# imperatormk/candle-birefnet

Hardware: AMD Instinct MI355X
Metric: images/sec @1024x1024 Swin-L (higher is better)
Workload: dtype f32 storage+accumulate; GEMM operands as two fp16 planes of the power-of-two-scaled operand (22-bit mantissa), 3 fp16 MFMAs/product (fp32-equivalent inside the fp16 range: |GEMM input| < 8190); 1 GPU; BASELINE configs[1]: Swin-L 1024x1024 batch=1 fp32 on 1xMI355X (single-image latency); batch_per_gpu=1, global_batch=1, size=1024, deform_mode=reference_cpu, compute=f32_half2, streams_per_gpu=1, branch_streams_per_gpu=5, inputs=resident in HBM (torch cuda tensors), weights: synthetic seed 42

## Files before the change

### candle_birefnet_amd/_ffi.py

```python
import ctypes as C
import os

_HERE = os.path.dirname(os.path.abspath(__file__))
LIB_PATH = os.environ.get("BRN_LIB_PATH") or os.path.join(_HERE, "libbirefnet_hip.so")

BRN_OK = 0
BRN_MEM_HOST, BRN_MEM_DEVICE = 0, 1
BRN_F32, BRN_F32_SPLIT3, BRN_F32_SPLIT2, BRN_BF16_OPERANDS, BRN_BF16, BRN_BF16_DEC_SPLIT2, BRN_F32_HALF2, BRN_F16 = 0, 1, 2, 3, 4, 5, 6, 7
BRN_DEFORM_REFERENCE_CPU, BRN_DEFORM_DEFORMABLE = 0, 1
BRN_ACT_NONE, BRN_ACT_RELU, BRN_ACT_GELU_ERF = 0, 1, 2

BRN_ERR_INVALID_ARG, BRN_ERR_MISSING_TENSOR, BRN_ERR_SHAPE, BRN_ERR_NO_DEVICE, BRN_ERR_HIP, BRN_ERR_OOM = 1, 2, 3, 4, 5, 6
ERR_NAMES = {1: "INVALID_ARG", 2: "MISSING_TENSOR", 3: "SHAPE", 4: "NO_DEVICE", 5: "HIP", 6: "OOM"}


class BrnError(RuntimeError):

    def __init__(self, status, msg):
        super().__init__(f"[{ERR_NAMES.get(status, status)}] {msg}")
        self.status = status


class brn_config(C.Structure):
    _fields_ = [
# ... 7 lines not shown
        ("deform_mode", C.c_int),
    ]


class brn_named_tensor(C.Structure):
    _fields_ = [("name", C.c_char_p), ("data", C.POINTER(C.c_float)), ("shape", C.POINTER(C.c_int64)), ("ndim", C.c_int)]


def _load():
    if not os.path.exists(LIB_PATH):
        raise ImportError(
            f"{LIB_PATH} not found: build it with `python -c 'import __graft_entry__ as g; g.build()'` "
            "(hipcc --offload-arch=gfx950).  There is no CPU fallback for this package.")
    return C.CDLL(LIB_PATH, mode=C.RTLD_GLOBAL)


lib = _load()

_fp = C.POINTER(C.c_float)
_vp = C.c_void_p


def _sig(name, restype, *argtypes):
    fn = getattr(lib, name)
    fn.restype = restype
    fn.argtypes = list(argtypes)
    return fn


_sig("brn_abi_version", C.c_int)
_sig("brn_last_error", C.c_char_p)
_sig("brn_build_info", C.c_char_p)
_sig("brn_device_count", C.c_int, C.POINTER(C.c_int))
_sig("brn_config_default_swin_l", None, C.POINTER(brn_config))
_sig("brn_config_lateral_channels", None, C.POINTER(brn_config), C.POINTER(C.c_int * 4))
_sig("brn_config_x4_channels", C.c_int, C.POINTER(brn_config))
_sig("brn_model_create", C.c_int, C.POINTER(brn_config), C.POINTER(brn_named_tensor), C.c_size_t, C.c_int, C.c_int,
     C.c_int, C.c_int, C.c_int, C.POINTER(_vp))
_sig("brn_model_create_from_safetensors", C.c_int, C.POINTER(brn_config), C.c_char_p, C.c_char_p, C.c_int, C.c_int, C.c_int,
     C.c_int, C.c_int, C.POINTER(_vp))
_sig("brn_decoder_create", C.c_int, C.POINTER(brn_config), C.POINTER(brn_named_tensor), C.c_size_t, C.c_char_p, C.c_int, C.c_int, C.POINTER(_vp))
_sig("brn_model_destroy", None, _vp)
_sig("brn_forward_logits", C.c_int, _vp, _vp, C.c_int, C.c_int, C.c_int, C.c_int, _vp, C.c_int, _vp)
_sig("brn_forward", C.c_int, _vp, _vp, C.c_int, C.c_int, C.c_int, C.c_int, _vp, C.c_int, _vp)
_sig("brn_model_backbone_forward", C.c_int, _vp, _vp, C.c_int, C.c_int, C.c_int, C.c_int, C.POINTER(_vp), C.c_int, _vp)
_sig("brn_model_squeeze_forward", C.c_int, _vp, _vp, C.c_int, C.c_int, C.c_int, C.c_int, _vp, C.c_int, _vp)
_sig("brn_model_decoder_forward", C.c_int, _vp, _vp, _vp, _vp, _vp, _vp, C.c_int, C.c_int, C.c_int, C.c_int, _vp, C.c_int, _vp)
_sig("brn_model_set_streams", C.c_int, _vp, C.c_int, C.c_int)
_sig("brn_model_set_profiling", C.c_int, _vp, C.c_int)
_sig("brn_model_last_timings", C.c_int, _vp, C.POINTER(C.c_float * 5))
_sig("brn_model_last_kernel_stats", C.c_int, _vp, C.c_int, C.POINTER(C.c_int), C.POINTER(C.c_float), C.POINTER(C.c_double),
     C.POINTER(C.c_double), C.POINTER(C.c_int))
_sig("brn_kernel_family_name", C.c_char_p, C.c_int)
_sig("brn_swin_create", C.c_int, C.POINTER(brn_config), C.POINTER(brn_named_tensor), C.c_size_t, C.c_char_p, C.c_int,
     C.POINTER(_vp))
_sig("brn_swin_destroy", None, _vp)
_sig("brn_swin_forward", C.c_int, _vp, _vp, C.c_int, C.c_int, C.c_int, C.c_int, C.POINTER(_vp), C.c_int, _vp)
_sig("brn_linear_forward", C.c_int, _vp, C.c_int, C.c_int, _vp, _vp, C.c_int, C.c_int, _vp, _vp, C.c_int, C.c_int, _vp)
_sig("brn_linear_residual_layer_norm_forward", C.c_int, _vp, C.c_int, C.c_int, _vp, _vp, C.c_int, _vp, _vp, _vp, C.c_float, _vp, _vp, C.c_int, C.c_int, _vp)
_sig("brn_layer_norm_forward", C.c_int, _vp, C.c_int, C.c_int, _vp, _vp, C.c_float, _vp, C.c_int, C.c_int, _vp)
_sig("brn_conv2d_forward", C.c_int, _vp, C.c_int, C.c_int, C.c_int, C.c_int, _vp, _vp, C.c_int, C.c_int, C.c_int, C.c_int,
     C.c_int, C.c_int, _vp, _vp, _vp, _vp, C.c_float, C.c_int, _vp, C.c_int, C.c_int, _vp)
_sig("brn_upsample_bilinear2d", C.c_int, _vp, C.c_int, C.c_int, C.c_int, C.c_int, C.c_int, C.c_int, _vp, C.c_int, C.c_int, _vp)
_sig("brn_window_attention_forward", C.c_int, _vp, C.c_int, C.c_int, C.c_int, C.c_int, C.c_int, C.c_int, C.c_int, _vp, _vp,
     _vp, _vp, _vp, _vp, C.c_int, C.c_int, _vp)
_sig("brn_patch_merging_forward", C.c_int, _vp, C.c_int, C.c_int, C.c_int, C.c_int, _vp, _vp, _vp, _vp, C.c_int, C.c_int, _vp)
_sig("brn_deform_conv2d_forward", C.c_int, _vp, C.c_int, C.c_int, C.c_int, C.c_int, _vp, _vp, _vp, _vp, _vp, _vp, C.c_int,
     C.c_int, C.c_int, C.c_int, C.c_int, _vp, C.c_int, C.c_int, _vp)

_sig("brn_aspp_deformable_forward", C.c_int, _vp, C.c_size_t, C.c_char_p, C.c_int, C.c_int, C.c_int, _vp, C.c_int, C.c_int, C.c_int, _vp, C.c_int, C.c_int, _vp)

_sig("brn_decblk_forward", C.c_int, _vp, C.c_size_t, C.c_char_p, C.c_int, C.c_int, C.c_int, C.c_int, C.c_int, _vp, C.c_int, C.c_int, C.c_int, _vp, C.c_int,
     C.c_int, _vp)

_sig("brn_preprocess_image", C.c_int, _vp, C.c_int, C.c_int, C.c_int, C.c_int, _vp, C.c_int, C.c_int, _vp)
_sig("brn_postprocess_mask", C.c_int, _vp, C.c_int, C.c_int, C.c_int, C.c_int, C.c_int, _vp, C.c_int, _vp)
_sig("brn_infer_images_u8", C.c_int, _vp, C.c_int, C.POINTER(_vp), C.POINTER(C.c_int), C.POINTER(C.c_int), C.c_int, C.c_int, C.POINTER(_vp), _vp)
_sig("brn_set_op_compute", C.c_int, C.c_int)
if hasattr(lib, "brn_gemm_microbench"):
    _sig("brn_gemm_microbench", C.c_int, C.c_int, C.c_int, C.c_int, C.c_int, C.c_int, C.c_int, C.c_int, C.POINTER(C.c_float))

DECLARED = [
    "brn_abi_version", "brn_last_error", "brn_build_info", "brn_device_count", "brn_config_default_swin_l",
    "brn_config_lateral_channels", "brn_config_x4_channels", "brn_model_create", "brn_model_create_from_safetensors", "brn_decoder_create", "brn_model_destroy", "brn_forward_logits",
    "brn_forward", "brn_model_backbone_forward", "brn_model_squeeze_forward", "brn_model_decoder_forward",
    "brn_model_set_streams", "brn_model_set_profiling", "brn_model_last_timings", "brn_model_last_kernel_stats", "brn_kernel_family_name",
    "brn_swin_create", "brn_swin_destroy", "brn_swin_forward", "brn_linear_forward", "brn_linear_residual_layer_norm_forward", "brn_layer_norm_forward",
    "brn_conv2d_forward", "brn_upsample_bilinear2d", "brn_window_attention_forward", "brn_patch_merging_forward",
    "brn_deform_conv2d_forward", "brn_aspp_deformable_forward", "brn_decblk_forward", "brn_set_op_compute", "brn_preprocess_image", "brn_postprocess_mask", "brn_infer_images_u8",
]


def check(status):
    if status != BRN_OK:
        raise BrnError(status, (lib.brn_last_error() or b"").decode("utf-8", "replace"))


def device_count():
    n = C.c_int(0)
    check(lib.brn_device_count(C.byref(n)))
    return n.value
```

### candle_birefnet_amd/csrc/brn_api.cpp

```cpp
#include "brn_api_util.h"
#include <cstring>
#include <cstdio>
#include <memory>
#include <cstdlib>

namespace brn {

ComputeMode compute_mode(int dt) {
    ComputeMode m;
    if (dt == BRN_F32) m.build.planes = 0;
    else if (dt == BRN_F32_SPLIT3) m.build.planes = 3;
    else if (dt == BRN_F32_SPLIT2) m.build.planes = 2;
    else if (dt == BRN_F32_HALF2) m.build.planes = BUILD_HALF2;
#ifdef BRN_DIAG_BUILD
    else if (dt == BRN_BF16_OPERANDS) m.build.planes = 1;
#else
    else if (dt == BRN_BF16_OPERANDS) fail(BRN_ERR_INVALID_ARG, "compute dtype BRN_BF16_OPERANDS is superseded by BRN_BF16 and only built into libbirefnet_hip_diag.so");
#endif
    else if (dt == BRN_BF16 || dt == BRN_BF16_DEC_SPLIT2 || dt == BRN_F16) { m.build = {BUILD_BF16, dt == BRN_F16}; m.s16 = dt == BRN_F16 ? 2 : 1; }
    else fail(BRN_ERR_INVALID_ARG, "unsupported compute dtype %d", dt);
    return m;
}

static void plan_model(Model& m, int B, int H, int W) {
// ... 340 lines not shown
    delete m;
}

brn_status brn_forward_logits(brn_model* m, const float* x, int B, int H, int W, brn_mem in_loc, float* out, brn_mem out_loc,
                              void* stream) {
    return guarded([&] { run_model(m ? &m->m : nullptr, x, B, H, W, in_loc, out, out_loc, stream, 0); });
}
brn_status brn_forward(brn_model* m, const float* x, int B, int H, int W, brn_mem in_loc, float* out, brn_mem out_loc,
                       void* stream) {
    return guarded([&] { run_model(m ? &m->m : nullptr, x, B, H, W, in_loc, out, out_loc, stream, 1); });
}

brn_status brn_model_set_streams(brn_model* m, int sub_batch_streams, int branch_stream_mask) {
    return guarded([&] {
        if (!m) fail(BRN_ERR_INVALID_ARG, "null model");
        if (sub_batch_streams < 0 || sub_batch_streams > 8 || branch_stream_mask < -1 || branch_stream_mask > 31)
            fail(BRN_ERR_INVALID_ARG, "sub_batch_streams in 0 .. 8 (0 = default), branch_stream_mask in -1 .. 31 (-1 = automatic)");
        std::lock_guard<std::mutex> lk(m->m.mu);
        m->m.opt_parts = sub_batch_streams;
        m->m.opt_branches = branch_stream_mask;
    });
}
brn_status brn_model_set_profiling(brn_model* m, int enable) {
    return guarded([&] {
        if (!m) fail(BRN_ERR_INVALID_ARG, "null model");
        std::lock_guard<std::mutex> lk(m->m.mu);
        m->m.profiling = enable != 0;
    });
}
brn_status brn_model_last_timings(brn_model* m, float ms[5]) {
    return guarded([&] {
        if (!m || !ms) fail(BRN_ERR_INVALID_ARG, "null argument");
        for (int i = 0; i < 5; ++i) ms[i] = m->m.last_ms[i];
    });
}
brn_status brn_model_last_kernel_stats(brn_model* m, int n, int* launches, float* ms, double* flop, double* bytes, int* n_out) {
    return guarded([&] {
        if (!m || !launches || !ms || !flop || !bytes) fail(BRN_ERR_INVALID_ARG, "null argument");
        const int rows = FAM_COUNT + REGION_COUNT;
        const int k = n < rows ? n : rows;
        for (int f = 0; f < k; ++f) {
            launches[f] = m->m.fam_launches[f]; ms[f] = m->m.fam_ms[f]; flop[f] = m->m.fam_flop[f]; bytes[f] = m->m.fam_bytes[f];
        }
        if (n_out) *n_out = rows;
    });
}
const char* brn_kernel_family_name(int f) {
    static const char* names[FAM_COUNT] = {"gemm_dense", "gemm_conv_nhwc", "gemm_gather_nchw", "gemm_deform_nhwc",
                                           "window_attention", "layernorm", "resize", "elementwise"};
    static const char* regions[REGION_COUNT] = {"region_none", "region_aspp"};
    if (f >= FAM_COUNT && f < FAM_COUNT + REGION_COUNT) return regions[f - FAM_COUNT];
    return (f >= 0 && f < FAM_COUNT) ? names[f] : "?";
}

brn_status brn_model_backbone_forward(brn_model* m, const float* x, int B, int H, int W, brn_mem in_loc, float* const outs[4],
                                      brn_mem out_loc, void* stream) {
    return guarded([&] {
        if (!m) fail(BRN_ERR_INVALID_ARG, "null model");
        if (m->m.decoder_only) fail(BRN_ERR_INVALID_ARG, "this handle holds only the decoder (brn_decoder_create)");
        std::lock_guard<std::mutex> lk(m->m.mu);
        swin_entry(m->m.swin, m->m.device, x, B, H, W, in_loc, outs, out_loc, stream, m->m.bf16);
    });
}

brn_status brn_model_squeeze_forward(brn_model* m, const float* x4, int B, int h, int w, brn_mem in_loc, float* out,
                                     brn_mem out_loc, void* stream) {
    return guarded([&] {
        if (!m || !x4 || !out) fail(BRN_ERR_INVALID_ARG, "null argument");
        if (m->m.decoder_only) fail(BRN_ERR_INVALID_ARG, "this handle holds only the decoder (brn_decoder_create)");
        std::lock_guard<std::mutex> lk(m->m.mu);
        BRN_HIP(hipSetDevice(m->m.device));
        const int cin = m->m.squeeze.cin, cout = m->m.squeeze.cout;
        Staging si(stream, in_loc), so(stream, out_loc);
        const float* dx = si.in(x4, (size_t)B * cin * h * w);
        float* dy = so.out(out, (size_t)B * cout * h * w);
        with_arena((hipStream_t)stream, [&](Ctx& c) {
            Map X = new_map(c, B, h, w, cin), Y = new_map(c, B, h, w, cout);
            if (!c.dry) BRN_HIP(launch_nchw_to_nhwc(dx, B, cin, h, w, X.p, X.ld, 0, c.stream, c.bf16));
            decblk_forward(c, m->m.squeeze, X, Y, m->m.cfg.deform_mode);
            if (!c.dry) BRN_HIP(launch_nhwc_to_nchw(Y.p, B, cout, h, w, Y.ld, 0, dy, c.stream, c.bf16));
        }, m->m.dec_bf16);
        so.finish();
    });
}

brn_status brn_model_decoder_forward(brn_model* m, const float* x, const float* x1, const float* x2, const float* x3,
                                     const float* x4, int B, int H, int W, brn_mem in_loc, float* out, brn_mem out_loc,
                                     void* stream) {
    return guarded([&] {
        if (!m || !x || !x1 || !x2 || !x3 || !x4 || !out) fail(BRN_ERR_INVALID_ARG, "null argument");
        if (H % 32 || W % 32 || H < 32 || W < 32) fail(BRN_ERR_INVALID_ARG, "H and W must be positive multiples of 32");
        std::lock_guard<std::mutex> lk(m->m.mu);
        BRN_HIP(hipSetDevice(m->m.device));
        Staging si(stream, in_loc), so(stream, out_loc);
        const int hh[4] = {H / 4, H / 8, H / 16, H / 32}, ww[4] = {W / 4, W / 8, W / 16, W / 32};
        const int ch[4] = {384, 768, 1536, 3072};
        const float* src[4] = {x1, x2, x3, x4};
        const float* dsrc[4];
        for (int i = 0; i < 4; ++i) dsrc[i] = si.in(src[i], (size_t)B * ch[i] * hh[i] * ww[i]);
        const float* dx = si.in(x, (size_t)B * 3 * H * W);
        float* dy = so.out(out, (size_t)B * H * W);
        with_arena((hipStream_t)stream, [&](Ctx& c) {
            Map X1 = new_map(c, B, hh[0], ww[0], 384), X2 = new_map(c, B, hh[1], ww[1], 768), X3 = new_map(c, B, hh[2], ww[2], 1536);
            Map D4 = new_map(c, B, hh[3], ww[3], 3456);
            if (!c.dry) {
                BRN_HIP(launch_nchw_to_nhwc(dsrc[0], B, 384, hh[0], ww[0], X1.p, X1.ld, 0, c.stream, c.bf16));
// ... 12 lines not shown
```

### candle_birefnet_amd/csrc/brn_kernels.h

```cpp
#pragma once
#include <hip/hip_runtime.h>
#include <stdint.h>

namespace brn {

enum GemmMode {
    GEMM_DENSE = 0,
    GEMM_CONV_NHWC = 1,
    GEMM_GATHER_NCHW = 2,
    GEMM_DEFORM_NHWC = 3
};
enum Act { ACT_NONE = 0, ACT_RELU = 1, ACT_GELU_ERF = 2 };

struct GemmParams {
    const float* A;
    const float* W;
    float* C;
    int M, N, K;
    int mode;
    int lda;
    int a_coff;
    int Hin, Win, Cin, kh, kw, stride, pad, dil, Hout, Wout;
    int Kreal;
    const float* om; int om_ld; int om_mask_off;
    int om_sigmoid;
    const float* bias;
    const float* bbias; int bbias_rows;
    const float* scale; const float* shift;
    int act;
    const float* R; int ldr; int r_coff;
    int ldc; int c_coff;
    const void* Wp; int planes; int wp_rows;
    int splitk; float* part;
    int a_planes, c_planes;
    int h2; float a_scale, out_scale;
    int wp_ld;
    int k_chunk_major;
    int c_f32, r_f32;
    int a_bf16, c_bf16;
    unsigned long long* trace;
    int abl;
};

struct GemmPlan { int cfg; int splitk; size_t ws_floats; };
GemmPlan plan_gemm(int M, int N, int K, int planes = 0);
hipError_t launch_gemm(const GemmParams& p, const GemmPlan& plan, float* ws, hipStream_t s);
inline bool gemm_split_is_ws(int cfg) { return cfg == 6 || cfg == 0 || cfg == 3 || cfg == 4 || cfg == 5; }
hipError_t launch_gemm_split(const GemmParams& p, int cfg, hipStream_t s);

int launch_cus();
void set_launch_cus(int n);
GemmPlan plan_gemm_bf16(int M, int N, int K, bool f32_residual = false, bool gelu = false);
hipError_t launch_gemm_bf16(const GemmParams& p, const GemmPlan& plan, float* ws, hipStream_t s);

bool gemm_wstat_eligible(const GemmParams& p);
hipError_t launch_gemm_wstat(const GemmParams& p, hipStream_t s);
bool patch_embed_ln_eligible(int Cin, int N, int k, int stride, int H, int W, int ldw, int ldx);
hipError_t launch_patch_embed_ln(const float* img, int B, int H, int W, const float* wgt, int ldw, const float* bias, const float* gamma,
                                 const float* beta, float eps, float* x, int ldx, hipStream_t s, const float* gamma1 = nullptr,
                                 const float* beta1 = nullptr, void* xn_bf16 = nullptr, int ldxn = 0, int xn_f16 = 0);
bool gemm_wstat_ln_eligible(const GemmParams& p);
bool gemm_rowln_eligible(const GemmParams& p);
hipError_t launch_gemm_rowln(const GemmParams& p, const float* gamma, const float* beta, float eps, void* y_bf16, int ldy, hipStream_t s);
hipError_t launch_gemm_wstat_ln(const GemmParams& p, const float* gamma, const float* beta, float eps, void* y_bf16, int ldy, hipStream_t s);

bool deform_bf16_eligible(const GemmParams& p);
hipError_t launch_deform_bf16(const GemmParams& p, hipStream_t s);

bool gemm_planes_eligible(const GemmParams& p);
GemmPlan plan_gemm_planes(int M, int N, int K, int planes, bool c_planes);
hipError_t launch_gemm_planes(const GemmParams& p, const GemmPlan& plan, float* ws, hipStream_t s);

namespace hf {
GemmPlan plan_gemm_bf16(int M, int N, int K, bool f32_residual = false, bool gelu = false);
hipError_t launch_gemm_bf16(const GemmParams& p, const GemmPlan& plan, float* ws, hipStream_t s);
bool gemm_wstat_eligible(const GemmParams& p);
hipError_t launch_gemm_wstat(const GemmParams& p, hipStream_t s);
bool gemm_wstat_ln_eligible(const GemmParams& p);
hipError_t launch_gemm_wstat_ln(const GemmParams& p, const float* gamma, const float* beta, float eps, void* y_bf16, int ldy, hipStream_t s);
bool gemm_rowln_eligible(const GemmParams& p);
hipError_t launch_gemm_rowln(const GemmParams& p, const float* gamma, const float* beta, float eps, void* y_bf16, int ldy, hipStream_t s);
bool deform_bf16_eligible(const GemmParams& p);
hipError_t launch_deform_bf16(const GemmParams& p, hipStream_t s);
}

#ifdef BRN_DIAG_BUILD
hipError_t launch_mfma_valu_probe(int blocks, int iters, int mode, float* sink, hipStream_t s);
hipError_t launch_lds_mfma_probe(int blocks, int iters, int np, int variant, float* sink, hipStream_t s);
hipError_t launch_mfma_peak_bf16(int blocks, int iters, float* sink, unsigned long long* clk, int nacc, hipStream_t s);
hipError_t launch_mfma_peak(int blocks, int iters, float* sink, unsigned long long* clk, hipStream_t s);
#endif

struct LayerNormParams {
    const float* x; float* y;
    int rows, C;
    const float* gamma; const float* beta; float eps;
    int ldx;
    int ldy, y_coff;
    int mode; int H, W, Cin;
    int y_planes;
    float y_h2;
// ... 53 lines not shown
```

### candle_birefnet_amd/csrc/kernels/gemm_f32.hip

```cpp
#include <cstdlib>
#include "../brn_kernels.h"
#include "gemm_common.h"

namespace brn {

constexpr int LDS_LD = 36;

template <int BM, int BN, int WM, int WN, int MODE>
__global__ void __launch_bounds__(WM* WN * 64) gemm_f32_kernel(const GemmParams p) {
    constexpr int NT = WM * WN * 64;
    constexpr int RPP = NT / 8;
    constexpr int PA = BM / RPP, PB = BN / RPP;
    constexpr int WTM = BM / WM, WTN = BN / WN, TM = WTM / 32, TN = WTN / 32;
    static_assert(PA >= 1 && PB >= 1 && TM >= 1 && TN >= 1, "tile too small for the thread count");

    constexpr int SMEM_MAIN = (BM + BN) * LDS_LD, SMEM_EPI = WM * WN * EPI_WAVE_FLOATS;
    __shared__ __attribute__((aligned(16))) float smem[SMEM_MAIN > SMEM_EPI ? SMEM_MAIN : SMEM_EPI];
    float* As = smem;
    float* Bs = smem + BM * LDS_LD;

    const int tid = threadIdx.x, lane = tid & 63, wave = tid >> 6;
    const int wm = wave / WN, wn = wave % WN;

    const TileSlice ts = tile_slice<BM, BN>(p, BK);
// ... 226 lines not shown
            pl.cfg = 0; pl.splitk = 1; pl.ws_floats = 0;
            static const int sk_t128 = getenv("BRN_SK_T128") ? atoi(getenv("BRN_SK_T128")) : 200;
            if (t128 < sk_t128) {
                int s = (int)(480 / t128);
                if (s > nk / 24) s = nk / 24;
                if (s > 8) s = 8;
                if (s > 1) { pl.splitk = s; pl.ws_floats = (size_t)s * M * N; }
            }
            return pl;
        }
    }
    if (t64 < 384 && nk >= 8) {
        pl.cfg = 2;
        int s = (int)((768 + t64 - 1) / t64);
        if (s > nk / 4) s = nk / 4;
        if (s > 64) s = 64;
        if (s > 1) { pl.splitk = s; pl.ws_floats = (size_t)s * M * N; }
    }
    return pl;
}

static bool deform_on_split(const GemmParams& p) {
    return p.mode == GEMM_DEFORM_NHWC && p.planes >= 2 && p.Wp && p.om && !p.a_bf16 && !p.c_bf16 && (p.Cin % 32) == 0 && p.K == p.kh * p.kw * p.Cin &&
           ((p.lda | p.a_coff) & 3) == 0 && p.Hin + p.pad < 32768 && p.Win + p.pad < 32768 &&
           ((double)p.M / ((double)p.Hout * p.Wout) + 1.0) * p.Hin * p.Win * p.lda * 4.0 < 2147483648.0;
}
static int deform_split_plan(const GemmParams& p, int caller_slices, int& splitk) {
    const GemmPlan pp = plan_gemm(p.M, p.N, p.K, p.planes);
    splitk = pp.splitk < caller_slices ? pp.splitk : caller_slices;
    if (splitk < 1) splitk = 1;
    return gemm_split_is_ws(pp.cfg) ? 0 : 2;
}

hipError_t launch_gemm(const GemmParams& p_in, const GemmPlan& pl, float* ws, hipStream_t s) {
    if (p_in.M <= 0 || p_in.N <= 0 || p_in.K <= 0 || (p_in.K % BK) != 0) return hipErrorInvalidValue;
    if ((p_in.mode == GEMM_CONV_NHWC || p_in.mode == GEMM_DEFORM_NHWC) && (p_in.Cin % BK) != 0) return hipErrorInvalidValue;
    GemmParams p = p_in;
    p.splitk = pl.splitk < 1 ? 1 : pl.splitk;
    p.part = ws;
    if (p.splitk > 1 && !ws) return hipErrorInvalidValue;
    if (p.a_bf16 && p.mode != GEMM_DEFORM_NHWC) return hipErrorInvalidValue;
    if (p.c_bf16 && (p.splitk > 1 || p.R || (p.planes > 0 && p.Wp && p.mode != GEMM_DEFORM_NHWC && p.mode != GEMM_GATHER_NCHW))) return hipErrorInvalidValue;
    const bool deform_split = deform_on_split(p);
    int deform_cfg = 0;
    if (deform_split) deform_cfg = deform_split_plan(p, p.splitk, p.splitk);
    if (p.h2 && !(p.planes == 2 && p.Wp && (p.mode == GEMM_DENSE || p.mode == GEMM_CONV_NHWC || deform_split))) p.h2 = 0;
    if (p.h2 && !(p.a_scale > 0.f && p.out_scale > 0.f)) return hipErrorInvalidValue;
    if (p.a_planes || p.c_planes) {
        if (!(p.planes == 2 || p.planes == 3) || !p.Wp || p.mode != GEMM_DENSE || !gemm_split_is_ws(pl.cfg)) return hipErrorInvalidValue;
        if (p.a_planes && (p.a_planes != p.planes || p.lda % 16 || p.a_coff)) return hipErrorInvalidValue;
        if (p.c_planes && (p.c_planes != p.planes || p.splitk > 1 || p.R || p.N % 32 || p.ldc % 16 || p.c_coff % 32)) return hipErrorInvalidValue;
    }
    hipError_t e;
    if (p.planes > 0 && p.Wp && (p.mode == GEMM_DENSE || p.mode == GEMM_CONV_NHWC)) e = launch_gemm_split(p, pl.cfg, s);
    else if (deform_split) e = launch_gemm_split(p, deform_cfg, s);
    else if (pl.cfg == 0) e = launch_cfg<128, 128, 2, 2>(p, s);
    else if (pl.cfg == 1) e = launch_cfg<128, 64, 2, 2>(p, s);
    else if (pl.cfg == 3) e = launch_cfg<128, 128, 2, 4>(p, s);
    else if (pl.cfg == 4) e = launch_cfg<256, 128, 4, 2>(p, s);
    else if (pl.cfg == 5) e = launch_cfg<128, 128, 4, 2>(p, s);
    else e = launch_cfg<64, 64, 2, 2>(p, s);
    if (e != hipSuccess || p.splitk == 1) return e;
    long total = (long)p.M * p.N;
    long blocks = (total + 255) / 256;
    if (blocks > 4096) blocks = 4096;
    hipLaunchKernelGGL(splitk_reduce_kernel, dim3((unsigned)blocks), dim3(256), 0, s, p);
    return hipGetLastError();
}

}
```

### include/birefnet_hip.h

```cpp
#ifndef BIREFNET_HIP_H
#define BIREFNET_HIP_H

#include <stddef.h>
#include <stdint.h>

#ifdef __cplusplus
extern "C" {
#endif

#define BRN_ABI_VERSION 1

typedef int brn_status;
enum {
    BRN_OK = 0,
    BRN_ERR_INVALID_ARG = 1,
    BRN_ERR_MISSING_TENSOR = 2,
    BRN_ERR_SHAPE = 3,
    BRN_ERR_NO_DEVICE = 4,
    BRN_ERR_HIP = 5,
    BRN_ERR_OOM = 6
};

typedef enum { BRN_MEM_HOST = 0, BRN_MEM_DEVICE = 1 } brn_mem;
typedef enum { BRN_F32 = 0, BRN_F32_SPLIT3 = 1, BRN_F32_SPLIT2 = 2, BRN_BF16_OPERANDS = 3, BRN_BF16 = 4, BRN_BF16_DEC_SPLIT2 = 5, BRN_F32_HALF2 = 6, BRN_F16 = 7 } brn_dtype;
// ... 22 lines not shown
    int deform_mode;
} brn_config;

typedef struct brn_named_tensor {
    const char* name;
    const float* data;
    const int64_t* shape;
    int ndim;
} brn_named_tensor;

typedef struct brn_model brn_model;
typedef struct brn_swin brn_swin;

int brn_abi_version(void);
const char* brn_last_error(void);
brn_status brn_device_count(int* n);
const char* brn_build_info(void);

void brn_config_default_swin_l(brn_config* cfg);
void brn_config_lateral_channels(const brn_config* cfg, int out[4]);
int brn_config_x4_channels(const brn_config* cfg);

brn_status brn_model_create(const brn_config* cfg, const brn_named_tensor* weights, size_t n_weights,
                            int device_ordinal, brn_dtype compute_dtype,
                            int max_batch, int max_h, int max_w, brn_model** out);
brn_status brn_model_create_from_safetensors(const brn_config* cfg, const char* path, const char* prefix,
                                            int device_ordinal, brn_dtype compute_dtype,
                                            int max_batch, int max_h, int max_w, brn_model** out);
void brn_model_destroy(brn_model* m);

brn_status brn_forward_logits(brn_model* m, const float* x_nchw, int B, int H, int W, brn_mem in_loc,
                              float* logits_out, brn_mem out_loc, void* stream);
brn_status brn_forward(brn_model* m, const float* x_nchw, int B, int H, int W, brn_mem in_loc,
                       float* mask_out, brn_mem out_loc, void* stream);

brn_status brn_model_backbone_forward(brn_model* m, const float* x_nchw, int B, int H, int W, brn_mem in_loc,
                                      float* const outs[4], brn_mem out_loc, void* stream);
brn_status brn_model_squeeze_forward(brn_model* m, const float* x4_nchw, int B, int h, int w, brn_mem in_loc,
                                     float* out, brn_mem out_loc, void* stream);
brn_status brn_model_decoder_forward(brn_model* m, const float* x_nchw, const float* x1, const float* x2,
                                     const float* x3, const float* x4, int B, int H, int W, brn_mem in_loc,
                                     float* logits_out, brn_mem out_loc, void* stream);

brn_status brn_decoder_create(const brn_config* cfg, const brn_named_tensor* weights, size_t n_weights, const char* prefix,
                              int device_ordinal, brn_dtype compute_dtype, brn_model** out);

brn_status brn_model_set_streams(brn_model* m, int sub_batch_streams, int branch_stream_mask);

brn_status brn_model_set_profiling(brn_model* m, int enable);
brn_status brn_model_last_timings(brn_model* m, float ms[5]);
brn_status brn_model_last_kernel_stats(brn_model* m, int n, int* launches, float* ms, double* flop,
                                       double* bytes, int* n_out);
const char* brn_kernel_family_name(int f);

brn_status brn_swin_create(const brn_config* cfg , const brn_named_tensor* weights,
                           size_t n_weights, const char* prefix, int device_ordinal, brn_swin** out);
void brn_swin_destroy(brn_swin* s);
brn_status brn_swin_forward(brn_swin* s, const float* x_nchw, int B, int H, int W, brn_mem in_loc,
                            float* const outs[4], brn_mem out_loc, void* stream);

brn_status brn_set_op_compute(int dtype);
brn_status brn_linear_forward(const float* x, int M, int K, const float* w, const float* bias, int N,
                              int act, const float* residual, float* y, brn_mem loc, int device_ordinal,
                              void* stream);
brn_status brn_linear_residual_layer_norm_forward(const float* x, int M, int K, const float* w, const float* bias, int N,
                                                  const float* residual, const float* gamma, const float* beta, float eps,
                                                  float* x_out, float* y_out, brn_mem loc, int device_ordinal, void* stream);

brn_status brn_layer_norm_forward(const float* x, int rows, int C, const float* gamma, const float* beta,
                                  float eps, float* y, brn_mem loc, int device_ordinal, void* stream);
brn_status brn_conv2d_forward(const float* x, int B, int C, int H, int W, const float* w, const float* bias,
                              int O, int kh, int kw, int stride, int pad, int dil,
                              const float* bn_gamma, const float* bn_beta, const float* bn_mean,
                              const float* bn_var, float bn_eps, int act,
                              float* y, brn_mem loc, int device_ordinal, void* stream);
brn_status brn_upsample_bilinear2d(const float* x, int B, int C, int H, int W, int out_h, int out_w,
                                   float* y, brn_mem loc, int device_ordinal, void* stream);
brn_status brn_window_attention_forward(const float* x, int B, int H, int W, int C, int heads, int window_size,
                                        int shift, const float* qkv_w, const float* qkv_b,
                                        const float* proj_w, const float* proj_b, const float* rel_table,
                                        float* y, brn_mem loc, int device_ordinal, void* stream);
brn_status brn_patch_merging_forward(const float* x, int B, int H, int W, int C, const float* norm_g,
                                     const float* norm_b, const float* reduction_w, float* y, brn_mem loc,
                                     int device_ordinal, void* stream);
brn_status brn_deform_conv2d_forward(const float* x, int B, int C, int H, int W,
                                     const float* offset_w, const float* offset_b,
                                     const float* mod_w, const float* mod_b,
                                     const float* w, const float* bias, int O, int k, int stride, int pad,
                                     int mode, float* y, brn_mem loc, int device_ordinal, void* stream);

brn_status brn_aspp_deformable_forward(const brn_named_tensor* weights, size_t n_weights, const char* prefix, int in_channels,
                                       int out_channels, int mode, const float* x, int B, int H, int W, float* y, brn_mem loc,
                                       int device_ordinal, void* stream);

brn_status brn_decblk_forward(const brn_named_tensor* weights, size_t n_weights, const char* prefix, int in_channels,
                              int out_channels, int inter_channels, int use_aspp, int mode, const float* x, int B, int H, int W,
                              float* y, brn_mem loc, int device_ordinal, void* stream);

brn_status brn_preprocess_image(const unsigned char* pixels, int h, int w, int channels, int S,
                                float* x_nchw_out, brn_mem out_loc, int device_ordinal, void* stream);
brn_status brn_postprocess_mask(const float* logits, int S, brn_mem in_loc, int apply_sigmoid, int out_h, int out_w,
                                unsigned char* mask_out, int device_ordinal, void* stream);

brn_status brn_infer_images_u8(brn_model* m, int n, const unsigned char* const* pixels, const int* heights, const int* widths,
                               int channels, int S, unsigned char* const* masks, void* stream);

// ... 5 lines not shown
```

### rust_shim/src/hip_ffi.rs

```rust
#![allow(non_camel_case_types)]
use libc::{c_char, c_double, c_float, c_int, c_uchar, c_void, size_t};

pub const BRN_ABI_VERSION: c_int = 1;
pub const BRN_OK: c_int = 0;
pub const BRN_MEM_HOST: c_int = 0;
pub const BRN_MEM_DEVICE: c_int = 1;
pub const BRN_F32: c_int = 0;
pub const BRN_F32_SPLIT3: c_int = 1;
pub const BRN_F32_SPLIT2: c_int = 2;
pub const BRN_BF16_OPERANDS: c_int = 3;
pub const BRN_BF16: c_int = 4;
pub const BRN_BF16_DEC_SPLIT2: c_int = 5;
pub const BRN_F32_HALF2: c_int = 6;
pub const BRN_F16: c_int = 7;
pub const BRN_DEFORM_REFERENCE_CPU: c_int = 0;
pub const BRN_DEFORM_DEFORMABLE: c_int = 1;
pub const BRN_ACT_NONE: c_int = 0;
pub const BRN_ACT_RELU: c_int = 1;
pub const BRN_ACT_GELU_ERF: c_int = 2;

#[repr(C)]
#[derive(Clone, Copy)]
pub struct BrnConfig {
    pub size_w: c_int,
// ... 11 lines not shown
    pub num_heads: [c_int; 4],
    pub window_size: c_int,
    pub mlp_ratio: c_float,
    pub patch_size: c_int,
    pub in_channels: c_int,
    pub drop_path_rate: c_float,
    pub deform_mode: c_int,
}

#[repr(C)]
pub struct BrnNamedTensor {
    pub name: *const c_char,
    pub data: *const c_float,
    pub shape: *const i64,
    pub ndim: c_int,
}

pub enum BrnModel {}
pub enum BrnSwin {}

extern "C" {
    pub fn brn_abi_version() -> c_int;
    pub fn brn_last_error() -> *const c_char;
    pub fn brn_device_count(n: *mut c_int) -> c_int;
    pub fn brn_build_info() -> *const c_char;
    pub fn brn_config_default_swin_l(cfg: *mut BrnConfig);
    pub fn brn_config_lateral_channels(cfg: *const BrnConfig, out: *mut c_int);
    pub fn brn_config_x4_channels(cfg: *const BrnConfig) -> c_int;
    pub fn brn_model_create(cfg: *const BrnConfig, weights: *const BrnNamedTensor, n_weights: size_t, device_ordinal: c_int,
                            compute_dtype: c_int, max_batch: c_int, max_h: c_int, max_w: c_int, out: *mut *mut BrnModel) -> c_int;
    pub fn brn_model_create_from_safetensors(cfg: *const BrnConfig, path: *const c_char, prefix: *const c_char, device_ordinal: c_int,
                                             compute_dtype: c_int, max_batch: c_int, max_h: c_int, max_w: c_int,
                                             out: *mut *mut BrnModel) -> c_int;
    pub fn brn_decoder_create(cfg: *const BrnConfig, weights: *const BrnNamedTensor, n_weights: size_t, prefix: *const c_char,
                              device_ordinal: c_int, compute_dtype: c_int, out: *mut *mut BrnModel) -> c_int;
    pub fn brn_model_destroy(m: *mut BrnModel);
    pub fn brn_forward_logits(m: *mut BrnModel, x_nchw: *const c_float, b: c_int, h: c_int, w: c_int, in_loc: c_int,
                              logits_out: *mut c_float, out_loc: c_int, stream: *mut c_void) -> c_int;
    pub fn brn_forward(m: *mut BrnModel, x_nchw: *const c_float, b: c_int, h: c_int, w: c_int, in_loc: c_int,
                       mask_out: *mut c_float, out_loc: c_int, stream: *mut c_void) -> c_int;
    pub fn brn_model_backbone_forward(m: *mut BrnModel, x_nchw: *const c_float, b: c_int, h: c_int, w: c_int, in_loc: c_int,
                                      outs: *const *mut c_float, out_loc: c_int, stream: *mut c_void) -> c_int;
    pub fn brn_model_squeeze_forward(m: *mut BrnModel, x4_nchw: *const c_float, b: c_int, h: c_int, w: c_int, in_loc: c_int,
                                     out: *mut c_float, out_loc: c_int, stream: *mut c_void) -> c_int;
    pub fn brn_model_decoder_forward(m: *mut BrnModel, x_nchw: *const c_float, x1: *const c_float, x2: *const c_float,
                                     x3: *const c_float, x4: *const c_float, b: c_int, h: c_int, w: c_int, in_loc: c_int,
                                     logits_out: *mut c_float, out_loc: c_int, stream: *mut c_void) -> c_int;
    pub fn brn_model_set_streams(m: *mut BrnModel, sub_batch_streams: c_int, branch_stream_mask: c_int) -> c_int;
    pub fn brn_model_set_profiling(m: *mut BrnModel, enable: c_int) -> c_int;
    pub fn brn_model_last_timings(m: *mut BrnModel, ms: *mut c_float) -> c_int;
    pub fn brn_model_last_kernel_stats(m: *mut BrnModel, n: c_int, launches: *mut c_int, ms: *mut c_float, flop: *mut c_double,
                                       bytes: *mut c_double, n_out: *mut c_int) -> c_int;
    pub fn brn_kernel_family_name(f: c_int) -> *const c_char;
    pub fn brn_swin_create(cfg: *const BrnConfig, weights: *const BrnNamedTensor, n_weights: size_t, prefix: *const c_char,
                           device_ordinal: c_int, out: *mut *mut BrnSwin) -> c_int;
    pub fn brn_swin_destroy(s: *mut BrnSwin);
    pub fn brn_swin_forward(s: *mut BrnSwin, x_nchw: *const c_float, b: c_int, h: c_int, w: c_int, in_loc: c_int,
                            outs: *const *mut c_float, out_loc: c_int, stream: *mut c_void) -> c_int;
    pub fn brn_set_op_compute(dtype: c_int) -> c_int;
    pub fn brn_linear_forward(x: *const c_float, m: c_int, k: c_int, w: *const c_float, bias: *const c_float, n: c_int, act: c_int,
                              residual: *const c_float, y: *mut c_float, loc: c_int, device_ordinal: c_int, stream: *mut c_void) -> c_int;
    pub fn brn_linear_residual_layer_norm_forward(x: *const c_float, m: c_int, k: c_int, w: *const c_float, bias: *const c_float, n: c_int,
                                                  residual: *const c_float, gamma: *const c_float, beta: *const c_float, eps: c_float,
                                                  x_out: *mut c_float, y_out: *mut c_float, loc: c_int, device_ordinal: c_int, stream: *mut c_void) -> c_int;
    pub fn brn_layer_norm_forward(x: *const c_float, rows: c_int, c: c_int, gamma: *const c_float, beta: *const c_float, eps: c_float,
                                  y: *mut c_float, loc: c_int, device_ordinal: c_int, stream: *mut c_void) -> c_int;
    pub fn brn_conv2d_forward(x: *const c_float, b: c_int, c: c_int, h: c_int, w: c_int, wgt: *const c_float, bias: *const c_float,
                              o: c_int, kh: c_int, kw: c_int, stride: c_int, pad: c_int, dil: c_int, bn_gamma: *const c_float,
                              bn_beta: *const c_float, bn_mean: *const c_float, bn_var: *const c_float, bn_eps: c_float, act: c_int,
                              y: *mut c_float, loc: c_int, device_ordinal: c_int, stream: *mut c_void) -> c_int;
    pub fn brn_upsample_bilinear2d(x: *const c_float, b: c_int, c: c_int, h: c_int, w: c_int, out_h: c_int, out_w: c_int,
                                   y: *mut c_float, loc: c_int, device_ordinal: c_int, stream: *mut c_void) -> c_int;
    pub fn brn_window_attention_forward(x: *const c_float, b: c_int, h: c_int, w: c_int, c: c_int, heads: c_int, window_size: c_int,
                                        shift: c_int, qkv_w: *const c_float, qkv_b: *const c_float, proj_w: *const c_float,
                                        proj_b: *const c_float, rel_table: *const c_float, y: *mut c_float, loc: c_int,
                                        device_ordinal: c_int, stream: *mut c_void) -> c_int;
    pub fn brn_patch_merging_forward(x: *const c_float, b: c_int, h: c_int, w: c_int, c: c_int, norm_g: *const c_float,
                                     norm_b: *const c_float, reduction_w: *const c_float, y: *mut c_float, loc: c_int,
                                     device_ordinal: c_int, stream: *mut c_void) -> c_int;
    pub fn brn_deform_conv2d_forward(x: *const c_float, b: c_int, c: c_int, h: c_int, w: c_int, offset_w: *const c_float,
                                     offset_b: *const c_float, mod_w: *const c_float, mod_b: *const c_float, wgt: *const c_float,
                                     bias: *const c_float, o: c_int, k: c_int, stride: c_int, pad: c_int, mode: c_int, y: *mut c_float,
                                     loc: c_int, device_ordinal: c_int, stream: *mut c_void) -> c_int;
    pub fn brn_aspp_deformable_forward(weights: *const BrnNamedTensor, n_weights: usize, prefix: *const c_char, in_channels: c_int,
                                       out_channels: c_int, mode: c_int, x: *const c_float, b: c_int, h: c_int, w: c_int, y: *mut c_float,
                                       loc: c_int, device_ordinal: c_int, stream: *mut c_void) -> c_int;
    pub fn brn_decblk_forward(weights: *const BrnNamedTensor, n_weights: usize, prefix: *const c_char, in_channels: c_int, out_channels: c_int,
                              inter_channels: c_int, use_aspp: c_int, mode: c_int, x: *const c_float, b: c_int, h: c_int, w: c_int, y: *mut c_float, loc: c_int,
                              device_ordinal: c_int, stream: *mut c_void) -> c_int;
    pub fn brn_preprocess_image(pixels: *const c_uchar, h: c_int, w: c_int, channels: c_int, s: c_int, x_nchw_out: *mut c_float,
                                out_loc: c_int, device_ordinal: c_int, stream: *mut c_void) -> c_int;
    pub fn brn_infer_images_u8(m: *mut BrnModel, n: c_int, pixels: *const *const c_uchar, heights: *const c_int, widths: *const c_int, channels: c_int,
                               s: c_int, masks: *const *mut c_uchar, stream: *mut c_void) -> c_int;
    pub fn brn_postprocess_mask(logits: *const c_float, s: c_int, in_loc: c_int, apply_sigmoid: c_int, out_h: c_int, out_w: c_int,
                                mask_out: *mut c_uchar, device_ordinal: c_int, stream: *mut c_void) -> c_int;
}

pub(crate) struct ModelHandle(pub(crate) *mut BrnModel);
unsafe impl Send for ModelHandle {}
unsafe impl Sync for ModelHandle {}
impl Drop for ModelHandle {
    fn drop(&mut self) {
        unsafe { brn_model_destroy(self.0) }
    }
}

// ... 37 lines not shown
```

Baseline: 94.09 images/s.

## Add weight-stationary persistent split-plane GEMM for large-M K=192 dense layers

Adds a persistent GEMM kernel that keeps the whole split-plane weight slice (192 columns × K) in registers for each wave. It streams 32-row A tiles through double-buffered LDS with buffer_load_lds, then stages the fp32 C tile through the same LDS for a coalesced epilogue. Work is spread across XCDs by row ranges. It is enabled by default only for K=192 dense GEMMs with M ≥ 81920, which are the stage-1 Swin linears at 1024px. The aim is to stop re-fetching weights per tile and to overlap A loads with MFMA work, at the cost of high register pressure and a narrow eligibility path.

```diff
diff --git a/candle_birefnet_amd/_ffi.py b/candle_birefnet_amd/_ffi.py
--- a/candle_birefnet_amd/_ffi.py
+++ b/candle_birefnet_amd/_ffi.py
@@ -83,6 +83,8 @@
 _sig("brn_model_last_kernel_stats", C.c_int, _vp, C.c_int, C.POINTER(C.c_int), C.POINTER(C.c_float), C.POINTER(C.c_double),
      C.POINTER(C.c_double), C.POINTER(C.c_int))
 _sig("brn_kernel_family_name", C.c_char_p, C.c_int)
+if hasattr(lib, "brn_wstat_split_launch_count"):
+    _sig("brn_wstat_split_launch_count", C.c_int)
 _sig("brn_swin_create", C.c_int, C.POINTER(brn_config), C.POINTER(brn_named_tensor), C.c_size_t, C.c_char_p, C.c_int,
      C.POINTER(_vp))
 _sig("brn_swin_destroy", None, _vp)
@@ -115,7 +117,7 @@
     "brn_abi_version", "brn_last_error", "brn_build_info", "brn_device_count", "brn_config_default_swin_l",
     "brn_config_lateral_channels", "brn_config_x4_channels", "brn_model_create", "brn_model_create_from_safetensors", "brn_decoder_create", "brn_model_destroy", "brn_forward_logits",
     "brn_forward", "brn_model_backbone_forward", "brn_model_squeeze_forward", "brn_model_decoder_forward",
-    "brn_model_set_streams", "brn_model_set_profiling", "brn_model_last_timings", "brn_model_last_kernel_stats", "brn_kernel_family_name",
+    "brn_model_set_streams", "brn_model_set_profiling", "brn_model_last_timings", "brn_model_last_kernel_stats", "brn_kernel_family_name", "brn_wstat_split_launch_count",
     "brn_swin_create", "brn_swin_destroy", "brn_swin_forward", "brn_linear_forward", "brn_linear_residual_layer_norm_forward", "brn_layer_norm_forward",
     "brn_conv2d_forward", "brn_upsample_bilinear2d", "brn_window_attention_forward", "brn_patch_merging_forward",
     "brn_deform_conv2d_forward", "brn_aspp_deformable_forward", "brn_decblk_forward", "brn_set_op_compute", "brn_preprocess_image", "brn_postprocess_mask", "brn_infer_images_u8",
diff --git a/candle_birefnet_amd/csrc/brn_api.cpp b/candle_birefnet_amd/csrc/brn_api.cpp
--- a/candle_birefnet_amd/csrc/brn_api.cpp
+++ b/candle_birefnet_amd/csrc/brn_api.cpp
@@ -416,6 +416,8 @@
     if (f >= FAM_COUNT && f < FAM_COUNT + REGION_COUNT) return regions[f - FAM_COUNT];
     return (f >= 0 && f < FAM_COUNT) ? names[f] : "?";
 }
+
+int brn_wstat_split_launch_count(void) { return (int)brn::gemm_wstat_split_launches(); }
 
 brn_status brn_model_backbone_forward(brn_model* m, const float* x, int B, int H, int W, brn_mem in_loc, float* const outs[4],
                                       brn_mem out_loc, void* stream) {
diff --git a/candle_birefnet_amd/csrc/brn_kernels.h b/candle_birefnet_amd/csrc/brn_kernels.h
--- a/candle_birefnet_amd/csrc/brn_kernels.h
+++ b/candle_birefnet_amd/csrc/brn_kernels.h
@@ -47,6 +47,9 @@
 hipError_t launch_gemm(const GemmParams& p, const GemmPlan& plan, float* ws, hipStream_t s);
 inline bool gemm_split_is_ws(int cfg) { return cfg == 6 || cfg == 0 || cfg == 3 || cfg == 4 || cfg == 5; }
 hipError_t launch_gemm_split(const GemmParams& p, int cfg, hipStream_t s);
+bool gemm_wstat_split_eligible(const GemmParams& p);
+hipError_t launch_gemm_wstat_split(const GemmParams& p, hipStream_t s);
+long gemm_wstat_split_launches();
 
 int launch_cus();
 void set_launch_cus(int n);
diff --git a/candle_birefnet_amd/csrc/kernels/gemm_f32.hip b/candle_birefnet_amd/csrc/kernels/gemm_f32.hip
--- a/candle_birefnet_amd/csrc/kernels/gemm_f32.hip
+++ b/candle_birefnet_amd/csrc/kernels/gemm_f32.hip
@@ -302,7 +302,8 @@
         if (p.c_planes && (p.c_planes != p.planes || p.splitk > 1 || p.R || p.N % 32 || p.ldc % 16 || p.c_coff % 32)) return hipErrorInvalidValue;
     }
     hipError_t e;
-    if (p.planes > 0 && p.Wp && (p.mode == GEMM_DENSE || p.mode == GEMM_CONV_NHWC)) e = launch_gemm_split(p, pl.cfg, s);
+    if (gemm_wstat_split_eligible(p)) e = launch_gemm_wstat_split(p, s);
+    else if (p.planes > 0 && p.Wp && (p.mode == GEMM_DENSE || p.mode == GEMM_CONV_NHWC)) e = launch_gemm_split(p, pl.cfg, s);
     else if (deform_split) e = launch_gemm_split(p, deform_cfg, s);
     else if (pl.cfg == 0) e = launch_cfg<128, 128, 2, 2>(p, s);
     else if (pl.cfg == 1) e = launch_cfg<128, 64, 2, 2>(p, s);
diff --git a/candle_birefnet_amd/csrc/kernels/wstat_split_gemm.hip b/candle_birefnet_amd/csrc/kernels/wstat_split_gemm.hip
--- /dev/null
+++ b/candle_birefnet_amd/csrc/kernels/wstat_split_gemm.hip
@@ -0,0 +1,201 @@
+#include "../brn_kernels.h"
+#include "gemm_common.h"
+#include <atomic>
+#include <cstdlib>
+
+namespace brn {
+
+__device__ __forceinline__ int wss_slot(int r, int c) { return (r >> 1) * 256 + (((((r & 1) << 3) | c) ^ ((r >> 1) & 15)) << 4); }
+__device__ __forceinline__ void wss_blds16(__amdgpu_buffer_rsrc_t rsrc, unsigned voff, int soff, void* lds_dst) {
+    __builtin_amdgcn_raw_ptr_buffer_load_lds(rsrc, (__attribute__((address_space(3))) void*)lds_dst, 16, voff, soff, 0, 0);
+}
+template <int N> __device__ __forceinline__ void wss_wait_vmcnt() { asm volatile("s_waitcnt vmcnt(%0)" ::"n"(N) : "memory"); }
+
+template <int N, int S> __device__ __forceinline__ void wss_wait_vmcnt_k(int k) {
+    if (k >= 2) wss_wait_vmcnt<N + 2 * S>(); else if (k == 1) wss_wait_vmcnt<N + S>(); else wss_wait_vmcnt<N>();
+}
+template <int AHEAD, int NI, int S>
+__device__ __forceinline__ void wss_wait_landed(int n, int k) {
+    static_assert(AHEAD >= 1 && AHEAD <= 2 && AHEAD * NI + 2 * S <= 63, "vmcnt is a 6-bit counter");
+    if (n <= 0) { wss_wait_vmcnt<0>(); return; }
+    if constexpr (AHEAD == 2) { if (n >= 2) { wss_wait_vmcnt_k<2 * NI, S>(k); return; } }
+    wss_wait_vmcnt_k<NI, S>(k);
+}
+
+template <int KT, int NW, int WGPC, int NBUF, bool H>
+__global__ void __launch_bounds__(NW * 64, (NW * WGPC + 3) / 4) gemm_wstat_split_kernel(const GemmParams p) {
+    constexpr int WBM = 32, WBN = 192, SUB = WBM * 128;
+    constexpr int ABUF = KT * SUB;
+    constexpr int CPW = WBN / NW, NB = CPW / 16;
+    constexpr int NI = 4 * KT / NW;
+    constexpr int NT = NW * 64, CH_ROW = WBN / 4;
+    constexpr int PASSES = NT >= 384 ? 1 : 2, LPR = NT * PASSES / WBM, CPL = CH_ROW / LPR;
+    static_assert(CPW * NW == WBN && NB * 16 == CPW && NI * NW == 4 * KT && LPR * CPL == CH_ROW && LPR * WBM == NT * PASSES, "geometry");
+    static_assert(ABUF >= WBM * WBN * 4, "the fp32 C tile must fit the A buffer it replaces");
+    __shared__ __attribute__((aligned(1024))) char smem[NBUF * ABUF];
+    const int tid = threadIdx.x, lane = tid & 63;
+    const int wave = __builtin_amdgcn_readfirstlane(tid >> 6);
+    const int G = p.N / WBN, T = (p.M + WBM - 1) / WBM;
+    const int xcd = blockIdx.x & 7, li = blockIdx.x >> 3, nw = ((int)gridDim.x >> 3) / G;
+    const int grp = li % G, wk = li / G;
+    const int t_lo = (int)((long)T * xcd / 8), t_hi = (int)((long)T * (xcd + 1) / 8);
+    if (wk >= nw || t_lo + wk >= t_hi) return;
+    const int n0 = grp * WBN + wave * CPW;
+    bf16x8 wfr[NB][KT][2];
+    {
+        const char* wp = reinterpret_cast<const char*>(p.Wp) + ((long)(n0 + (lane & 15)) * KT * 2) * 64 + (lane >> 4) * 16;
+#pragma unroll
+        for (int j = 0; j < NB; ++j)
+#pragma unroll
+            for (int kt = 0; kt < KT; ++kt)
+#pragma unroll
+                for (int pl = 0; pl < 2; ++pl) wfr[j][kt][pl] = *reinterpret_cast<const bf16x8*>(wp + ((long)(16 * j * KT + kt) * 2 + pl) * 64);
+    }
+    const int er = tid / LPR, ec = tid - er * LPR;
+    EpiCols cols[CPL];
+#pragma unroll
+    for (int k = 0; k < CPL; ++k) {
+        cols[k].split = false; cols[k].vec = true; cols[k].part = nullptr;
+        cols[k].sc = f32x4{1.f, 1.f, 1.f, 1.f}; cols[k].sh = zero4();
+        cols[k].bias = p.bias ? *reinterpret_cast<const f32x4*>(p.bias + grp * WBN + (ec + LPR * k) * 4) : zero4();
+    }
+#pragma unroll
+    for (int j = 0; j < NB; ++j)
+#pragma unroll
+        for (int kt = 0; kt < KT; ++kt)
+#pragma unroll
+            for (int pl = 0; pl < 2; ++pl) asm volatile("" : "+v"(wfr[j][kt][pl]));
+#pragma unroll
+    for (int k = 0; k < CPL; ++k) asm volatile("" : "+v"(cols[k].bias));
+    const float* Ab = p.A;
+    auto issue = [&](int t, char* buf) {
+        const int m0 = t * WBM;
+        __amdgpu_buffer_rsrc_t rs = __builtin_amdgcn_make_buffer_rsrc(const_cast<float*>(Ab + (long)m0 * p.lda), 0, 0x7fffffff, 0x00020000);
+#pragma unroll
+        for (int j = 0; j < NI; ++j) {
+            const int q = wave + NW * j, piece = q >> 2, ii = q & 3;
+            const int pr = 4 * ii + (lane >> 4), qs = (lane & 15) ^ (pr & 15);
+            const int row = 2 * pr + (qs >> 3);
+            const unsigned ro = (unsigned)((min(m0 + row, p.M - 1) - m0) * p.lda * 4) + (unsigned)((qs & 7) * 16);
+            wss_blds16(rs, ro, piece * 128, buf + piece * SUB + ii * 1024);
+        }
+    };
+    int a_foff[2][2];
+#pragma unroll
+    for (int i = 0; i < 2; ++i)
+#pragma unroll
+        for (int pl = 0; pl < 2; ++pl) a_foff[i][pl] = wss_slot(16 * i + (lane & 15), 4 * pl + (lane >> 4));
+
+    auto mfma_tile = [&](const char* buf, f32x4 (&acc)[2][NB]) {
+#pragma unroll
+        for (int i = 0; i < 2; ++i)
+#pragma unroll
+            for (int j = 0; j < NB; ++j) acc[i][j] = zero4();
+#pragma unroll
+        for (int kt = 0; kt < KT; ++kt) {
+            bf16x8 af[2][2];
+#pragma unroll
+            for (int pl = 0; pl < 2; ++pl)
+#pragma unroll
+                for (int i = 0; i < 2; ++i) af[pl][i] = *reinterpret_cast<const bf16x8*>(buf + kt * SUB + a_foff[i][pl]);
+#pragma unroll
+            for (int pr = 0; pr < 3; ++pr) {
+                const int pa = pr == 1 ? 1 : 0, pb = pr == 0 ? 1 : 0;
+#pragma unroll
+                for (int j = 0; j < NB; ++j)
+#pragma unroll
+                    for (int i = 0; i < 2; ++i) {
+                        if constexpr (H) acc[i][j] = __builtin_amdgcn_mfma_f32_16x16x32_f16(__builtin_bit_cast(f16x8, wfr[j][kt][pb]), __builtin_bit_cast(f16x8, af[pa][i]), acc[i][j], 0, 0, 0);
+                        else acc[i][j] = __builtin_amdgcn_mfma_f32_16x16x32_bf16(wfr[j][kt][pb], af[pa][i], acc[i][j], 0, 0, 0);
+                    }
+            }
+        }
+    };
+    const int epi_ops = (p.c_planes || p.R) ? 2 : 1;
+    int t = t_lo + wk;
+    constexpr int AHEAD = NBUF - 1, S_EPI = PASSES * CPL;
+#pragma unroll
+    for (int a = 0; a < AHEAD; ++a)
+        if (t + a * nw < t_hi) issue(t + a * nw, smem + a * ABUF);
+    int bi = 0, prev_ops = 0;
+    for (; t < t_hi; t += nw) {
+        char* buf = smem + bi * ABUF;
+        const int bn = bi + AHEAD >= NBUF ? bi + AHEAD - NBUF : bi + AHEAD;
+        if (t + AHEAD * nw < t_hi) issue(t + AHEAD * nw, smem + bn * ABUF);
+        const int rem = (t_hi - 1 - t) / nw;
+        wss_wait_landed<AHEAD, NI, S_EPI>(rem < AHEAD ? rem : AHEAD, prev_ops);
+        __builtin_amdgcn_s_barrier();
+        f32x4 acc[2][NB];
+        mfma_tile(buf, acc);
+        asm volatile("s_waitcnt lgkmcnt(0)" ::: "memory");
+        __builtin_amdgcn_s_barrier();
+#pragma unroll
+        for (int i = 0; i < 2; ++i) {
+            const int row = 16 * i + (lane & 15);
+#pragma unroll
+            for (int j = 0; j < NB; ++j) {
+                const int ch = (wave * CPW + 16 * j) / 4 + (lane >> 4);
+                *reinterpret_cast<f32x4*>(buf + row * (WBN * 4) + ((ch ^ (row & 15)) << 4)) = acc[i][j];
+            }
+        }
+        asm volatile("s_waitcnt lgkmcnt(0)" ::: "memory");
+        __builtin_amdgcn_s_barrier();
+        const int m0 = t * WBM;
+#pragma unroll
+        for (int ps = 0; ps < PASSES; ++ps) {
+            const int row = er + ps * (WBM / PASSES), m = m0 + row;
+            if (m < p.M) {
+#pragma unroll
+                for (int k = 0; k < CPL; ++k) {
+                    const int ch = ec + LPR * k;
+                    const f32x4 v = *reinterpret_cast<const f32x4*>(buf + row * (WBN * 4) + ((ch ^ (row & 15)) << 4));
+                    epilogue_row<false, true>(p, cols[k], m, grp * WBN + ch * 4, v);
+                }
+            }
+        }
+        asm volatile("s_waitcnt lgkmcnt(0)" ::: "memory");
+        __builtin_amdgcn_s_barrier();
+        prev_ops = m0 + WBM <= p.M ? epi_ops : 0;
+        bi = bi + 1 == NBUF ? 0 : bi + 1;
+    }
+}
+
+constexpr int WSTAT_SPLIT_DEFAULT_MASK = 1, WSTAT_SPLIT_DEFAULT_MIN_M = 81920;
+static int wstat_split_mask() {
+    static const int v = getenv("BRN_WSTAT_SPLIT") ? atoi(getenv("BRN_WSTAT_SPLIT")) : WSTAT_SPLIT_DEFAULT_MASK;
+    return v;
+}
+static int wstat_split_min_m() {
+    static const int v = getenv("BRN_WSTAT_SPLIT_MIN_M") ? atoi(getenv("BRN_WSTAT_SPLIT_MIN_M")) : WSTAT_SPLIT_DEFAULT_MIN_M;
+    return v;
+}
+static std::atomic<long> g_wstat_split_launches{0};
+long gemm_wstat_split_launches() { return g_wstat_split_launches.load(); }
+
+static int wstat_split_wgpc(int K) { return K == 192 ? 2 : 1; }
+bool gemm_wstat_split_eligible(const GemmParams& p) {
+    if (!(p.K == 192 ? (wstat_split_mask() & 1) : p.K == 384 ? (wstat_split_mask() & 2) : 0)) return false;
+    return p.mode == GEMM_DENSE && p.Wp && p.planes == 2 && p.a_planes == 2 && p.splitk == 1 && p.M >= wstat_split_min_m() &&
+           p.N >= 192 && (p.N % 192) == 0 && p.N / 192 <= launch_cus() * wstat_split_wgpc(p.K) / 8 &&
+           !p.scale && !p.bbias && !p.a_bf16 && !p.c_bf16 && !p.trace && !p.abl && p.a_coff == 0 && (p.lda % 16) == 0 && p.lda >= p.K &&
+           ((p.ldc | p.c_coff) & 3) == 0 && (!p.R || ((p.ldr | p.r_coff) & 3) == 0) && (!p.bias || ((size_t)p.bias & 15) == 0) &&
+           (!p.c_planes || (p.c_planes == 2 && !p.R)) && (long)p.lda * 4 * 32 < 0x7fffffffL;
+}
+template <int KT, int NW, int WGPC, int NBUF>
+static hipError_t launch_wstat_split_k(const GemmParams& p, hipStream_t s) {
+    const int G = p.N / 192;
+    const int nw = (launch_cus() * WGPC / 8) / G;
+    if (nw < 1) return hipErrorInvalidValue;
+    const dim3 grid(8 * G * nw), block(NW * 64);
+    if (p.h2) hipLaunchKernelGGL((gemm_wstat_split_kernel<KT, NW, WGPC, NBUF, true>), grid, block, 0, s, p);
+    else hipLaunchKernelGGL((gemm_wstat_split_kernel<KT, NW, WGPC, NBUF, false>), grid, block, 0, s, p);
+    g_wstat_split_launches.fetch_add(1);
+    return hipGetLastError();
+}
+hipError_t launch_gemm_wstat_split(const GemmParams& p, hipStream_t s) {
+    if (!gemm_wstat_split_eligible(p)) return hipErrorInvalidValue;
+    if (p.K == 192) return launch_wstat_split_k<6, 4, 2, 2>(p, s);
+    return launch_wstat_split_k<12, 4, 1, 2>(p, s);
+}
+
+}
diff --git a/include/birefnet_hip.h b/include/birefnet_hip.h
--- a/include/birefnet_hip.h
+++ b/include/birefnet_hip.h
@@ -98,6 +98,7 @@
 brn_status brn_model_last_kernel_stats(brn_model* m, int n, int* launches, float* ms, double* flop,
                                        double* bytes, int* n_out);
 const char* brn_kernel_family_name(int f);
+int brn_wstat_split_launch_count(void);
 
 brn_status brn_swin_create(const brn_config* cfg , const brn_named_tensor* weights,
                            size_t n_weights, const char* prefix, int device_ordinal, brn_swin** out);
diff --git a/rust_shim/src/hip_ffi.rs b/rust_shim/src/hip_ffi.rs
--- a/rust_shim/src/hip_ffi.rs
+++ b/rust_shim/src/hip_ffi.rs
@@ -87,6 +87,7 @@
     pub fn brn_model_last_kernel_stats(m: *mut BrnModel, n: c_int, launches: *mut c_int, ms: *mut c_float, flop: *mut c_double,
                                        bytes: *mut c_double, n_out: *mut c_int) -> c_int;
     pub fn brn_kernel_family_name(f: c_int) -> *const c_char;
+    pub fn brn_wstat_split_launch_count() -> c_int;
     pub fn brn_swin_create(cfg: *const BrnConfig, weights: *const BrnNamedTensor, n_weights: size_t, prefix: *const c_char,
                            device_ordinal: c_int, out: *mut *mut BrnSwin) -> c_int;
     pub fn brn_swin_destroy(s: *mut BrnSwin);
```

Result: no change. 94.73 images/s, median of 2 (+0.7%).
